# opensensor/thingino-accel

Hardware: AMD Instinct MI355X
Metric: images/sec yolov5s_int8 640x640 batch256 (higher is better)
Workload: dtype int8

## Files before the change

thingino-accel_amd/csrc/hip/conv_i8.hip:

```cpp
#include "conv_i8_common.hpp"

#ifndef I8M_ABL
#define I8M_ABL 0
#endif
template <int BPX, int BN, int STAGES, int KS = 1, int NW = 4>
__global__ __launch_bounds__(NW * 64) void conv_i8_mfma(const mhip_conv_i8_t p, const long total_pix, const int k64,
                                                         const int8_t *__restrict__ zeros, const unsigned noc,
                                                         const unsigned nblk, const int lg_inc, const unsigned kw_magic,
                                                         const fastdiv_t dhw, const fastdiv_t dow, const int bufmode,
                                                         const unsigned in_bytes) {
    ANAT_BEGIN();
    const bool POW2 = lg_inc >= 0;
    const bool masked = p.kh * p.kw <= 32;
    constexpr int SLICE = (BPX + BN) * BK;
    constexpr int STAGE = KS * SLICE;
    constexpr int NWN = BN == 128 ? 2 : 1;
    constexpr int NWM = NW / NWN;
    constexpr int WPX = BPX / NWM / 16;
    constexpr int WOC = BN / NWN / 16;
    constexpr int XROWS = BPX / NW;
    constexpr int XI = XROWS / 16;
    constexpr int LW = (BN / 16 + NW - 1) / NW;
    constexpr int L = XI + LW;
    static_assert(XI >= 1 && XROWS % 16 == 0, "every wave fetches whole 16-row pieces of the pixel tile");
    extern __shared__ __attribute__((aligned(16))) int8_t dynlds[];
    uint8_t *slut = (uint8_t *)dynlds;
    lds_base_must_be_zero(dynlds);
    long *rowoff = (long *)(dynlds + LUTB);
    int8_t *lds = dynlds + BPX * 8 + LUTB;

    const int tid = threadIdx.x, lane = tid & 63;
    const int wv = __builtin_amdgcn_readfirstlane(tid >> 6);
    const unsigned id = xcd_remap(blockIdx.x, nblk);
    const long pix0 = (long)(id / noc) * BPX;
    const int oc0 = (int)(id % noc) * BN;
    const int hw = p.out_h * p.out_w;

    const int wm = wv % NWM, wn = wv / NWM;
    const int pxw = wm * (WPX * 16), ocw = wn * (WOC * 16);
    v4i acc[WOC][WPX];
    init_acc<WPX, WOC>(p, acc, oc0 + ocw);
    if (p.lut2) { if (tid < 128) ((uint32_t *)slut)[tid] = ((const uint32_t *)p.lut2)[tid]; }
    else if (p.lut && tid < 64) ((uint32_t *)slut)[tid] = ((const uint32_t *)p.lut)[tid];
    fill_rowoff<BPX>(p, rowoff, [=](int row) { long q = pix0 + row; return q < total_pix ? q : -1L; }, (unsigned)hw, dhw);

    const int schunk = (lane & 3) ^ (((lane >> 4) & 1) << 1);
    const int8_t *xwin[XI];
    unsigned tapmask[XI];
    int iy0[XI], ix0[XI];
#pragma unroll
    for (int j = 0; j < XI; j++) {
        const long pix = pix0 + wv * XROWS + j * 16 + (lane >> 2);
        const bool valid = pix < total_pix;
        const unsigned f = valid ? fdiv((unsigned)pix, dhw) : 0u;
        const unsigned rem = valid ? (unsigned)pix - f * (unsigned)hw : 0u;
        const int oy = (int)fdiv(rem, dow), ox = (int)(rem - (unsigned)oy * (unsigned)p.out_w);
        iy0[j] = valid ? oy * p.stride_h - p.pad_top : -(1 << 28);
        ix0[j] = ox * p.stride_w - p.pad_left;
        xwin[j] = p.in + (size_t)f * p.in_stride + ((long)iy0[j] * p.in_w + ix0[j]) * p.in_c;
        unsigned m = 0;
        if (masked) {
            const int kx_lo = ix0[j] < 0 ? -ix0[j] : 0, kx_hi = p.in_w - ix0[j] < p.kw ? p.in_w - ix0[j] : p.kw;
            const unsigned colbits = kx_hi > kx_lo ? ((kx_hi >= 32 ? ~0u : (1u << kx_hi) - 1u) & ~((1u << kx_lo) - 1u)) : 0u;
            for (int r = 0; r < p.kh; r++) {
                const int iy = iy0[j] + r;
                if (iy >= 0 && iy < p.in_h) m |= colbits << (r * p.kw);
            }
// ... 57 lines not shown
#pragma unroll
        for (int j = 0; j < XI; j++) {
            bool ok;
            if (masked) {
                ok = kvalid & ((tapmask[j] >> tap) & 1u);
            } else {
                const int iy = iy0[j] + ky, ix = ix0[j] + kx;
                ok = kvalid & (iy >= 0) & (iy < p.in_h) & (ix >= 0) & (ix < p.in_w);
            }
            const int8_t *src = ok ? xwin[j] + koff : zeros;
            glds16(src, sb + (wv * XROWS + j * 16) * BK);
        }
#pragma unroll
        for (int j = 0; j < LW; j++) glds16(wsrc[j] + ks * BK, sb + BPX * BK + wq[j] * 16 * BK);
        if (!POW2) {
            rc += BK;
            while (rc >= p.in_c) { rc -= p.in_c; kx++; }
            while (kx >= p.kw) { kx -= p.kw; ky++; }
        }
    };

    const int nst = I8M_ABL & 2 ? 0 : nks / KS;
#pragma unroll
    for (int s = 0; s < STAGES - 1; s++)
        if (s < nst)
#pragma unroll
            for (int u = 0; u < KS; u++) issue(s * KS + u, s);

    const int frow = lane & 15, fchunk = lane >> 4;
    int stage = 0, nstage = STAGES - 1;
    ANAT_NOW(1);
    for (int st = 0; st < nst; st++) {
        const int ahead = nst - 1 - st;
        if (STAGES >= 4 && ahead >= 2) wait_vmcnt<2 * L * KS>();
        else if (STAGES >= 3 && ahead >= 1) wait_vmcnt<L * KS>();
        else wait_vmcnt<0>();
        __builtin_amdgcn_s_barrier();
        asm volatile("" ::: "memory");
#pragma unroll
        for (int u = 0; u < KS; u++) {
            const int8_t *xs = lds + stage * STAGE + u * SLICE, *ws = xs + BPX * BK;
            v4i xb[WPX], wa[WOC];
#pragma unroll
            for (int t = 0; t < WPX; t++) xb[t] = *(const v4i *)(xs + lds_off(pxw + t * 16 + frow, fchunk));
#pragma unroll
            for (int s = 0; s < WOC; s++) wa[s] = *(const v4i *)(ws + lds_off(ocw + s * 16 + frow, fchunk));
            if (u == 0 && st + STAGES - 1 < nst)
#pragma unroll
                for (int v = 0; v < KS; v++) issue((st + STAGES - 1) * KS + v, nstage);
#pragma unroll
            for (int s = 0; s < WOC; s++)
#pragma unroll
                for (int t = 0; t < WPX; t++) {
                    if (I8M_ABL & 4) asm volatile("" ::"v"(wa[s]), "v"(xb[t]));
                    else acc[s][t] = __builtin_amdgcn_mfma_i32_16x16x64_i8(wa[s], xb[t], acc[s][t], 0, 0, 0);
                }
        }
        stage = stage + 1 == STAGES ? 0 : stage + 1;
        nstage = nstage + 1 == STAGES ? 0 : nstage + 1;
    }
    ANAT_NOW(2);
    __syncthreads();
    if (I8M_ABL & 1) {
        int fold = 0;
#pragma unroll
        for (int s = 0; s < WOC; s++)
#pragma unroll
            for (int t = 0; t < WPX; t++) fold ^= acc[s][t][0] ^ acc[s][t][1] ^ acc[s][t][2] ^ acc[s][t][3];
        if (fold == 0x12345678) p.out[0] = 1;
        return;
    }
    epilogue<BPX, BN, WPX, WOC, true>(p, acc, lds, slut, rowoff, oc0, pxw, ocw, hw);
    ANAT_END(p);
}

__device__ __forceinline__ int lds_off128(int row, int chunk8) { return row * 128 + ((chunk8 ^ ((row >> 1) & 7)) << 4); }
template <int BPX, int BN, int NW>
__global__ __launch_bounds__(NW * 64) void conv_i8_r128(const mhip_conv_i8_t p, const long total_pix, const int k128,
                                                         const unsigned noc, const unsigned nblk, const int lg_inc,
                                                         const unsigned kw_magic, const fastdiv_t dhw, const fastdiv_t dow,
                                                         const unsigned in_bytes) {
    constexpr int STAGE = (BPX + BN) * 128;
    constexpr int NWN = BN == 128 ? 2 : 1;
    constexpr int NWM = NW / NWN;
    constexpr int WPX = BPX / NWM / 16;
    constexpr int WOC = BN / NWN / 16;
    constexpr int XI = BPX / 8 / NW;
    constexpr int WI = BN / 8 / NW;
    static_assert(XI >= 1 && WI >= 1 && BPX % (8 * NW) == 0 && BN % (8 * NW) == 0, "whole 8-row pieces per wave");
    extern __shared__ __attribute__((aligned(16))) int8_t dynlds[];
    uint8_t *slut = (uint8_t *)dynlds;
    lds_base_must_be_zero(dynlds);
    long *rowoff = (long *)(dynlds + LUTB);
    int8_t *lds = dynlds + BPX * 8 + LUTB;

    const int tid = threadIdx.x, lane = tid & 63;
    const int wv = __builtin_amdgcn_readfirstlane(tid >> 6);
    const unsigned id = xcd_remap(blockIdx.x, nblk);
    const long pix0 = (long)(id / noc) * BPX;
    const int oc0 = (int)(id % noc) * BN;
    const int hw = p.out_h * p.out_w;
    const int wm = wv % NWM, wn = wv / NWM;
    const int pxw = wm * (WPX * 16), ocw = wn * (WOC * 16);
    v4i acc[WOC][WPX];
    init_acc<WPX, WOC>(p, acc, oc0 + ocw);
    if (p.lut2) { if (tid < 128) ((uint32_t *)slut)[tid] = ((const uint32_t *)p.lut2)[tid]; }
    else if (p.lut && tid < 64) ((uint32_t *)slut)[tid] = ((const uint32_t *)p.lut)[tid];
    fill_rowoff<BPX>(p, rowoff, [=](int row) { long q = pix0 + row; return q < total_pix ? q : -1L; }, (unsigned)hw, dhw);

    const int lrow = lane >> 3, lslot = lane & 7;
    int xvoff[XI];
    unsigned tapmask[XI];
#pragma unroll
    for (int j = 0; j < XI; j++) {
        const int trow = (wv * XI + j) * 8 + lrow;
        const long pix = pix0 + trow;
        const bool valid = pix < total_pix;
        const unsigned f = valid ? fdiv((unsigned)pix, dhw) : 0u;
        const unsigned rem = valid ? (unsigned)pix - f * (unsigned)hw : 0u;
        const int oy = (int)fdiv(rem, dow), ox = (int)(rem - (unsigned)oy * (unsigned)p.out_w);
        const int iy0 = oy * p.stride_h - p.pad_top, ix0 = ox * p.stride_w - p.pad_left;
        const int chunk = lslot ^ ((trow >> 1) & 7);
        xvoff[j] = (int)(f * (unsigned)p.in_stride) + (iy0 * p.in_w + ix0) * p.in_c + chunk * 16;
        const int kx_lo = ix0 < 0 ? -ix0 : 0, kx_hi = p.in_w - ix0 < p.kw ? p.in_w - ix0 : p.kw;
        const unsigned colbits = kx_hi > kx_lo ? ((kx_hi >= 32 ? ~0u : (1u << kx_hi) - 1u) & ~((1u << kx_lo) - 1u)) : 0u;
        unsigned m = 0;
        for (int r = 0; r < p.kh; r++) {
            const int iy = iy0 + r;
            if (iy >= 0 && iy < p.in_h) m |= colbits << (r * p.kw);
        }
        tapmask[j] = valid ? m : 0u;
// ... 4 lines not shown
        const int trow = (wv * WI + j) * 8 + lrow;
        wvoff[j] = (oc0 + trow) * k128 + (lslot ^ ((trow >> 1) & 7)) * 16;
    }
    const __amdgpu_buffer_rsrc_t xrs = __builtin_amdgcn_make_buffer_rsrc((void *)p.in, 0, (int)in_bytes, 0x00020000);
    const __amdgpu_buffer_rsrc_t wrs = __builtin_amdgcn_make_buffer_rsrc((void *)p.w, 0, p.oc_pad * k128, 0x00020000);
    const int taps = p.kh * p.kw;
    const int nst = k128 / 128;
    auto issue = [&](int st, int buf) {
        int8_t *sb = lds + buf * STAGE;
        const int utap = (st * 128) >> lg_inc, urc = (st * 128) & ((1 << lg_inc) - 1);
        const int uky = (int)(((unsigned)utap * kw_magic) >> 16), ukx = utap - uky * p.kw;
        const int ukoff = (uky * p.in_w + ukx) * p.in_c + urc;
        const bool uvalid = utap < taps;
#pragma unroll
        for (int j = 0; j < XI; j++) {
            const bool ok = uvalid & (((tapmask[j] >> utap) & 1u) != 0u);
            blds16(xrs, ok ? xvoff[j] + ukoff : -1, 0, sb + (wv * XI + j) * 1024);
        }
#pragma unroll
        for (int j = 0; j < WI; j++) blds16(wrs, wvoff[j], st * 128, sb + BPX * 128 + (wv * WI + j) * 1024);
    };

    issue(0, 0);
    const int frow = lane & 15, fchunk = lane >> 4;
    for (int st = 0; st < nst; st++) {
        wait_vmcnt<0>();
        __builtin_amdgcn_s_barrier();
        asm volatile("" ::: "memory");
        const int8_t *xs = lds + (st & 1) * STAGE, *ws = xs + BPX * 128;
        v4i xb[2][WPX], wa[2][WOC];
#pragma unroll
        for (int h = 0; h < 2; h++) {
#pragma unroll
            for (int t = 0; t < WPX; t++) xb[h][t] = *(const v4i *)(xs + lds_off128(pxw + t * 16 + frow, h * 4 + fchunk));
#pragma unroll
            for (int q = 0; q < WOC; q++) wa[h][q] = *(const v4i *)(ws + lds_off128(ocw + q * 16 + frow, h * 4 + fchunk));
        }
        if (st + 1 < nst) issue(st + 1, (st + 1) & 1);
#pragma unroll
        for (int h = 0; h < 2; h++)
#pragma unroll
            for (int q = 0; q < WOC; q++)
#pragma unroll
                for (int t = 0; t < WPX; t++) acc[q][t] = __builtin_amdgcn_mfma_i32_16x16x64_i8(wa[h][q], xb[h][t], acc[q][t], 0, 0, 0);
    }
    __syncthreads();
    epilogue<BPX, BN, WPX, WOC, true>(p, acc, lds, slut, rowoff, oc0, pxw, ocw, hw);
}

template <int A, int B>
__device__ __forceinline__ void wait_vmcnt_at_most(int n) {
    constexpr int HI = A > B ? A : B, LO = A > B ? B : A;
    if (n >= A + B) wait_vmcnt<A + B>();
    else if (n >= HI) wait_vmcnt<HI>();
    else if (n >= LO) wait_vmcnt<LO>();
    else wait_vmcnt<0>();
}

struct conv_out_side_t {
    int8_t *out;
    size_t out_stride;
    const int8_t *w;
    const int32_t *bias;
    const uint8_t *lut, *lut2;
    int out_c, relu, out_pix_stride, out_ch_off;
    float cs;
    unsigned out_bytes;
};
template <int BPX, int BN, int STAGES, bool HAS_LUT, bool SEG = false, bool PAIR = false>
__global__ __launch_bounds__(NTHREADS) void conv_i8_persist(const mhip_conv_i8_t pin, const unsigned total_pix, const int k64,
                                                            const int8_t *__restrict__ zeros, const unsigned noc,
                                                            const unsigned npt, const unsigned ngrp, const int lg_inc,
                                                            const unsigned kw_magic, const fastdiv_t dhw, const fastdiv_t dow,
                                                            const unsigned out_bytes_first, const conv_out_side_t alt,
                                                            const unsigned noc0, const int bufmode, const unsigned in_bytes,
                                                            const int wres) {
    ANAT_BEGIN();
    const int STAGE = wres ? BPX * BK : (BPX + BN) * BK;
    constexpr int NWN = BN == 128 ? 2 : 1;
    constexpr int NWM = 4 / NWN;
    constexpr int WPX = BPX / NWM / 16;
    constexpr int WOC = BN / NWN / 16;
    constexpr int XI = BPX / 64;
    constexpr int LW = BN >= 128 ? 2 : 1;
    constexpr int L = XI + LW;
    constexpr int NST = WPX;
    extern __shared__ __attribute__((aligned(16))) int8_t dynlds[];
    uint8_t *slut = (uint8_t *)dynlds;
    int8_t *lds = dynlds + LUTB;
    lds_base_must_be_zero(dynlds);

    const int tid = threadIdx.x, lane = tid & 63;
    const int wv = __builtin_amdgcn_readfirstlane(tid >> 6);
    const unsigned id = xcd_remap(blockIdx.x, noc * ngrp);
    const unsigned grp = id / noc;
    unsigned ot = id - grp * noc;
    mhip_conv_i8_t p = pin;
    unsigned out_bytes = out_bytes_first;
    if (PAIR && ot >= noc0) {
        ot -= noc0;
        p.lut2 = alt.lut2;
        p.out = alt.out; p.out_stride = alt.out_stride; p.w = alt.w; p.bias = alt.bias; p.lut = alt.lut;
        p.out_c = alt.out_c; p.relu = alt.relu; p.out_pix_stride = alt.out_pix_stride; p.out_ch_off = alt.out_ch_off;
        p.cs = alt.cs;
        out_bytes = alt.out_bytes;
    }
    const int oc0 = (int)ot * BN;
    const unsigned t0 = (unsigned)(((unsigned long long)grp * npt) / ngrp);
    const unsigned t1 = (unsigned)(((unsigned long long)(grp + 1) * npt) / ngrp);
    if (t0 >= t1) return;
    const unsigned hw = (unsigned)(p.out_h * p.out_w);
    const int wm = wv % NWM, wn = wv / NWM;
    const int pxw = wm * (WPX * 16), ocw = wn * (WOC * 16);

    auto packed_row16 = [](int c) { return ((c >> 2) & 1) * 16 + (c >> 3) * 4 + (c & 3); };
    v4i bias[WOC];
#pragma unroll
    for (int s = 0; s < WOC; s++)
        bias[s] = p.bias ? *(const v4i *)(p.bias + (BN == 16 ? packed_row16((lane >> 4) * 4) : oc0 + ocw + s * 16 + (lane >> 4) * 4)) : (v4i){0, 0, 0, 0};
    if (HAS_LUT) {
        if (p.lut2) { if (tid < 128) ((uint32_t *)slut)[tid] = ((const uint32_t *)p.lut2)[tid]; }
        else if (tid < 64) ((uint32_t *)slut)[tid] = ((const uint32_t *)p.lut)[tid];
        __syncthreads();
    }
    const __amdgpu_buffer_rsrc_t orsrc = __builtin_amdgcn_make_buffer_rsrc(p.out, 0, (int)out_bytes, 0x00020000);

    const int schunk = (lane & 3) ^ (((lane >> 4) & 1) << 1);
    const int8_t *xwin[XI];
    unsigned tapmask[XI];
    unsigned rowf[SEG ? XI : 1], rowrem[SEG ? XI : 1];
    unsigned rowrem_up[SEG ? XI : 1];
    int xvoff[XI];
    auto setup_rows = [&](unsigned tile) {
#pragma unroll
        for (int j = 0; j < XI; j++) {
            const unsigned pix = tile * BPX + wv * (BPX / 4) + j * 16 + (lane >> 2);
            const bool valid = pix < total_pix;
            const unsigned f = valid ? fdiv(pix, dhw) : 0u;
            const unsigned rem = valid ? pix - f * hw : 0u;
            if (SEG) {
                rowf[j] = f;
                rowrem[j] = rem;
                const unsigned oy = fdiv(rem, dow), ox = rem - oy * (unsigned)p.out_w;
                rowrem_up[j] = (oy >> 1) * ((unsigned)p.out_w >> 1) + (ox >> 1);
                tapmask[j] = valid ? 1u : 0u;
                continue;
            }
// ... 81 lines not shown
        for (int ks = 0; ks < nks; ks++)
#pragma unroll
            for (int j = 0; j < LW; j++) glds16(wsrc[j] + ks * BK, wres_base + (ks * BN + wq[j] * 16) * BK);
    unsigned itile = t0;
    int iks = 0;
    int younger[STAGES - 1];
    setup_rows(t0);
    int nstage = 0;
#pragma unroll
    for (int s = 0; s < STAGES - 1; s++) {
        int n = 0;
        if (itile < t1) {
            issue(iks, nstage);
            n = wres ? XI : L;
            if (++iks == nks) {
                iks = 0;
                if (++itile < t1) setup_rows(itile);
            }
        }
#pragma unroll
        for (int i = 0; i < s; i++) younger[i] += n;
        younger[s] = 0;
        nstage++;
    }
    nstage = STAGES - 1;

    const int frow = lane & 15, fchunk = lane >> 4;
    const int chan = ocw + (lane >> 4) * (4 * WOC);
    const int pstride = p.out_pix_stride ? p.out_pix_stride : p.out_c;
    const int lo = p.relu ? 0 : -128;
    const uint8_t *lut128 = slut + 128;
    const bool ragged = (p.out_c % (WOC * 4)) != 0;
    int stage = 0;
    ANAT_NOW(1);
    for (unsigned tile = t0; tile < t1; tile++) {
        v4i acc[WOC][WPX];
        for (int ks = 0; ks < nks; ks++) {
            wait_vmcnt_at_most<(STAGES - 2) * L, NST>(younger[0]);
            __builtin_amdgcn_s_barrier();
            asm volatile("" ::: "memory");
            const int8_t *xs = lds + stage * STAGE, *ws = wres ? wres_base + ks * (BN * BK) : xs + BPX * BK;
            v4i xb[WPX], wa[WOC];
#pragma unroll
            for (int t = 0; t < WPX; t++) xb[t] = *(const v4i *)(xs + lds_off(pxw + t * 16 + frow, fchunk));
#pragma unroll
            for (int s = 0; s < WOC; s++) wa[s] = *(const v4i *)(ws + lds_off(ocw + s * 16 + frow, fchunk));
            int n = 0;
            if (itile < t1) {
                issue(iks, nstage);
                n = wres ? XI : L;
                if (++iks == nks) {
                    iks = 0;
                    if (++itile < t1) setup_rows(itile);
                }
            }
#pragma unroll
            for (int i = 0; i + 1 < STAGES - 1; i++) younger[i] = younger[i + 1] + n;
            younger[STAGES - 2] = 0;
            if (ks == 0) {
#pragma unroll
                for (int s = 0; s < WOC; s++)
#pragma unroll
                    for (int t = 0; t < WPX; t++) acc[s][t] = __builtin_amdgcn_mfma_i32_16x16x64_i8(wa[s], xb[t], bias[s], 0, 0, 0);
            } else {
#pragma unroll
                for (int s = 0; s < WOC; s++)
#pragma unroll
                    for (int t = 0; t < WPX; t++) acc[s][t] = __builtin_amdgcn_mfma_i32_16x16x64_i8(wa[s], xb[t], acc[s][t], 0, 0, 0);
            }
            stage = stage + 1 == STAGES ? 0 : stage + 1;
            nstage = nstage + 1 == STAGES ? 0 : nstage + 1;
        }
#ifdef ANATOMY
        if (tile + 1 == t1) ANAT_NOW(2);
#endif
#pragma unroll
        for (int t = 0; t < WPX; t++) {
            const unsigned pix = tile * BPX + pxw + t * 16 + (lane & 15);
            const unsigned f = fdiv(pix, dhw), rem = pix - f * hw;
            const unsigned off = f * (unsigned)p.out_stride + rem * (unsigned)pstride + (unsigned)(p.out_ch_off + oc0 + chan);
            const int nvalid = p.out_c - (oc0 + chan);
            const bool ok = pix < total_pix && nvalid >= WOC * 4;
// ... 217 lines not shown
        if (key && !strcmp(key, e.k)) {
            if (get) *get = *e.v;
            else *e.v = value;
            return 0;
        }
    return -1;
}
extern "C" int mhip_conv_i8_tune(const char *key, int value) { return tune_access(key, value, nullptr); }
extern "C" int mhip_conv_i8_tune_get(const char *key, int *value) { return value ? tune_access(key, 0, value) : -1; }

static int buf_mode(const mhip_conv_i8_t *p, int k64) {
    if (!tune().bufmode) return 0;
    return p->in_c >= 64 && (p->in_c & (p->in_c - 1)) == 0 && p->kh * p->kw <= 32 && (long)p->kh * p->kw * (p->kw - 1) < 65536 &&
           in_extent_bytes(p) <= 0x7fffffffL && (long)p->oc_pad * k64 <= 0x7fffffffL;
}

template <int BPX, int BN, int STAGES, int KS = 1, int NW = 4>
static int launch_mfma(const mhip_conv_i8_t *p, long total_pix, int k64) {
    const unsigned npt = (unsigned)((total_pix + BPX - 1) / BPX), noc = (unsigned)(p->oc_pad / BN);
    const unsigned nblk = npt * noc;
    const int nks = k64 / BK, nst = nks / KS, used = nst < STAGES ? nst : STAGES;
    if (KS > 1 && (nks % KS) != 0) return -1;
    size_t ring = (size_t)used * KS * (BPX + BN) * BK, tile = (size_t)BPX * (BN + OPAD);
    const size_t lds = BPX * 8 + LUTB + (ring > tile ? ring : tile);
    if (lds > 64 * 1024) {
        static bool attr = false;
        if (!attr && hipFuncSetAttribute((const void *)conv_i8_mfma<BPX, BN, STAGES, KS, NW>, hipFuncAttributeMaxDynamicSharedMemorySize,
                                         (int)(BPX * 8 + LUTB + (size_t)STAGES * KS * (BPX + BN) * BK)) != hipSuccess)
            return mhip_check(hipErrorUnknown, "conv_i8_mfma LDS attribute");
        attr = true;
    }
    int lg = -1;
    if ((p->in_c & (p->in_c - 1)) == 0 && (long)p->kh * p->kw * (p->kw - 1) < 65536) {
        lg = 0;
        while ((1 << lg) < p->in_c) lg++;
    }
    const unsigned magic = ((65536u + (unsigned)p->kw - 1u) / (unsigned)p->kw);
    hipLaunchKernelGGL((conv_i8_mfma<BPX, BN, STAGES, KS, NW>), dim3(nblk), dim3(NW * 64), lds, mhip_stream_native(), *p, total_pix,
                       k64, (const int8_t *)mhip_zero_page(), noc, nblk, lg, magic,
                       make_fastdiv((unsigned)(p->out_h * p->out_w)), make_fastdiv((unsigned)p->out_w),
                       lg >= 0 ? buf_mode(p, k64) : 0, (unsigned)in_extent_bytes(p));
    return mhip_check(hipGetLastError(), "conv_i8_mfma launch");
}


template <int BPX, int BN>
static size_t wres_lds(int k64) { return LUTB + 2 * (size_t)BPX * BK + (size_t)(k64 / BK) * BN * BK; }

template <int BPX, int BN, int STAGES, bool HAS_LUT, bool SEG = false, bool PAIR = false>
static int launch_persist_t(const mhip_conv_i8_t *p, long total_pix, int k64, int lg, unsigned magic,
                            const mhip_conv_i8_t *second = nullptr, int wres = 0) {
    if (BN == 16 && (p->out_c > 16 || p->oc_pad != 32 || (PAIR && (second->out_c > 16 || second->oc_pad != 32)))) return -1;
    const unsigned noc0 = BN == 16 ? 1u : (unsigned)(p->oc_pad / BN);
    const unsigned npt = (unsigned)((total_pix + BPX - 1) / BPX), noc = noc0 + (PAIR ? (BN == 16 ? 1u : (unsigned)(second->oc_pad / BN)) : 0u);
    conv_out_side_t alt;
    memset(&alt, 0, sizeof(alt));
    if (PAIR) {
        alt.out = second->out; alt.out_stride = second->out_stride; alt.w = second->w; alt.bias = second->bias;
        alt.lut = second->lut; alt.lut2 = second->lut2; alt.out_c = second->out_c; alt.relu = second->relu; alt.out_pix_stride = second->out_pix_stride;
        alt.out_ch_off = second->out_ch_off; alt.cs = second->cs;
    }
    if (PAIR) alt.out_bytes = (unsigned)persist_out_bytes(second);
    if (wres && STAGES != 2) return -1;
    const size_t lds = wres ? wres_lds<BPX, BN>(k64) : LUTB + (size_t)STAGES * (BPX + BN) * BK;
    if (wres) {
        static bool attr = false;
        if (!attr && hipFuncSetAttribute((const void *)conv_i8_persist<BPX, BN, STAGES, HAS_LUT, SEG, PAIR>,
                                         hipFuncAttributeMaxDynamicSharedMemorySize, 80 * 1024) != hipSuccess)
            return mhip_check(hipErrorUnknown, "conv_i8_persist LDS attribute");
        attr = true;
        int occ = 0, dev = 0;
        hipDeviceProp_t prop;
        if (hipOccupancyMaxActiveBlocksPerMultiprocessor(&occ, conv_i8_persist<BPX, BN, STAGES, HAS_LUT, SEG, PAIR>, NTHREADS, lds) != hipSuccess ||
            hipGetDevice(&dev) != hipSuccess || hipGetDeviceProperties(&prop, dev) != hipSuccess)
            return mhip_check(hipErrorUnknown, "conv_i8_persist occupancy query");
        unsigned g = (unsigned)((occ > 0 ? occ : 1) * prop.multiProcessorCount) / noc;
        if (tune().persist_slots > 0) g = (unsigned)tune().persist_slots / noc;
        if (g < 1) g = 1;
        if (g > npt) g = npt;
        hipLaunchKernelGGL((conv_i8_persist<BPX, BN, STAGES, HAS_LUT, SEG, PAIR>), dim3(noc * g), dim3(NTHREADS), lds,
                           mhip_stream_native(), *p, (unsigned)total_pix, k64, (const int8_t *)mhip_zero_page(), noc, npt, g, lg,
                           magic, make_fastdiv((unsigned)(p->out_h * p->out_w)), make_fastdiv((unsigned)p->out_w),
                           (unsigned)persist_out_bytes(p), alt, noc0, SEG ? 0 : buf_mode(p, k64), (unsigned)in_extent_bytes(p), 1);
        return mhip_check(hipGetLastError(), "conv_i8_persist (resident weights) launch");
    }
    static int slots = 0;
    if (!slots) {
// ... 29 lines not shown
}
static variant_t variant_of(int code) {
    if (code == 20) return variant_t{0, 0, 0, 0, 0, 0, 0, 0, 1};
    if (code == 18 || code == 19) return variant_t{0, 0, 0, 0, 0, 0, 0, code - 17, 0};
    if (code == 14 || code == 15) return variant_t{1, code == 15 ? 256 : 128, 2, 0, 0, 0, 1, 0, 0};
    if (code == 13) return variant_t{0, 256, 3, 0, 0, 1, 0, 0, 0};
    if (code == 12) return variant_t{0, 128, 2, 0, 1, 0, 0, 0, 0};
    if (code >= 9 && code <= 11) return variant_t{0, 0, 0, code == 10 ? 16 : (code == 9 ? 8 : 4), 0, 0, 0, 0, 0};
    if (code > 8 || code == 6 || code == 8) return variant_t{-1, 0, 0, 0, 0, 0, 0, 0, 0};
    const int c = code - 1;
    return variant_t{c & 1, (c & 2) ? 256 : 128, (c & 4) ? 3 : 2, 0, 0, 0, 0, 0, 0};
}

static bool r128_ok(const mhip_conv_i8_t *p) {
    const int C = p->in_c;
    return C >= 128 && (C & (C - 1)) == 0 && p->oc_pad % 128 == 0 && p->kh * p->kw <= 32 && (long)p->kh * p->kw * (p->kw - 1) < 65536 &&
           p->row_pad == p->kw * C && p->nseg <= 1 && in_extent_bytes(p) <= 0x7fffffffL && (long)p->oc_pad * p->kh * p->row_pad <= 0x7fffffffL;
}
template <int BPX, int BN, int NW>
static int launch_r128_t(const mhip_conv_i8_t *p, long total_pix) {
    const int k128 = p->kh * p->row_pad;
    const unsigned npt = (unsigned)((total_pix + BPX - 1) / BPX), noc = (unsigned)(p->oc_pad / BN);
    size_t ring = 2 * (size_t)(BPX + BN) * 128, tile = (size_t)BPX * (BN + OPAD);
    const size_t lds = BPX * 8 + LUTB + (ring > tile ? ring : tile);
    static bool attr = false;
    if (!attr && hipFuncSetAttribute((const void *)conv_i8_r128<BPX, BN, NW>, hipFuncAttributeMaxDynamicSharedMemorySize, (int)lds) != hipSuccess)
        return mhip_check(hipErrorUnknown, "conv_i8_r128 LDS attribute");
    attr = true;
    int lg = 0;
    while ((1 << lg) < p->in_c) lg++;
    const unsigned magic = ((65536u + (unsigned)p->kw - 1u) / (unsigned)p->kw);
    hipLaunchKernelGGL((conv_i8_r128<BPX, BN, NW>), dim3(npt * noc), dim3(NW * 64), lds, mhip_stream_native(), *p, total_pix, k128, noc,
                       npt * noc, lg, magic, make_fastdiv((unsigned)(p->out_h * p->out_w)), make_fastdiv((unsigned)p->out_w),
                       (unsigned)in_extent_bytes(p));
    return mhip_check(hipGetLastError(), "conv_i8_r128 launch");
}
static int launch_r128(const mhip_conv_i8_t *p, long total_pix, int form) {
    if (!r128_ok(p)) return -1;
    return form == 2 ? launch_r128_t<256, 128, 8>(p, total_pix) : launch_r128_t<128, 128, 4>(p, total_pix);
}
static bool seg_valid(const mhip_conv_i8_t *p) {
    if (p->nseg < 2 || p->nseg > 4 || p->kh != 1 || p->kw != 1 || p->stride_h != 1 || p->stride_w != 1 || p->pad_top ||
        p->pad_left || p->in_h != p->out_h || p->in_w != p->out_w)
        return false;
    int c = 0;
    if (p->seg_up && ((p->out_h | p->out_w) & 1)) return false;
    if (p->seg_up >> p->nseg) return false;
    for (int i = 0; i < 4; i++) {
        if (i < p->nseg) {
            if (!p->seg_in[i] || p->seg_c[i] <= 0 || (p->seg_c[i] & 31) || p->seg_c0[i] != c) return false;
            c += p->seg_c[i];
        } else if (p->seg_c0[i] != 0x7fffffff) {
            return false;
        }
    }
    return c == p->in_c;
}
static bool persist_eligible(const mhip_conv_i8_t *p) {
    if (p->add) return false;
    return !p->out_nchw && p->safe && (p->in_c & (p->in_c - 1)) == 0 && p->kh * p->kw <= 32 &&
           (long)p->kh * p->kw * (p->kw - 1) < 65536 && persist_out_bytes(p) <= 0x7fffffffL;
}
static bool wres_default(const mhip_conv_i8_t *p, int nks, int *bpx) {
    if (!tune().wres || p->kh * p->kw != 1 || p->in_c < 64 || p->out_h * p->out_w > 6400) return false;
    const int bn = p->oc_pad % 128 == 0 ? 128 : (p->oc_pad % 64 == 0 ? 64 : 32);
    const int px = (bn == 64 && p->out_h * p->out_w >= 6400) ? 256 : 128;
    if (LUTB + 2 * (size_t)px * BK + (size_t)nks * bn * BK > 80 * 1024) return false;
    *bpx = px;
    return true;
}

static variant_t default_variant(const mhip_conv_i8_t *p, int nks) {
    variant_t v;
    v.patch = 0;
    v.ks2 = 0;
    v.w8 = 0;
    v.wres = 0;
    v.r128 = 0;
    v.rows = 0;
    int ring = 0;
    const long wg_large = ((long)p->frames * p->out_h * p->out_w + 255) / 256 * ((p->oc_pad + 127) / 128);
    const bool few = wg_large < tune().few_wgs && tune().persist && !tune().bpx && !tune().stages && tune().small_batch;
    if (few) {
        if (conv_i8_patch_ok(p, 4, &ring)) {
            v.persist = 0; v.bpx = 0; v.stages = 0; v.patch = 4;
            return v;
        }
        if (nks >= 8 && r128_ok(p)) {
            v.persist = 0; v.bpx = 0; v.stages = 0; v.r128 = 1;
            return v;
// ... 133 lines not shown

extern "C" int mhip_conv_i8_variants(const mhip_conv_i8_t *p, int *codes, int max) {
    if (!p || (p->in_c % 16) != 0 || mhip_conv_i8_small_c(p->in_c, p->kw, p->out_c)) return 0;
    const int k64 = (p->kh * p->row_pad + BK - 1) / BK * BK, nks = k64 / BK;
    int n = 0;
    if (p->pre_w) {
        const int first = conv_i8_pre_tile_rows(p);
        for (int th : {first, 16, 8, 4})
            if (th && n < max && conv_i8_patch_ok(p, th, nullptr)) {
                const int code = th == 16 ? 10 : (th == 8 ? 9 : 11);
                bool seen = false;
                for (int i = 0; i < n; i++) seen |= codes[i] == code;
                if (!seen) codes[n++] = code;
            }
        return n;
    }
    if (p->nseg > 1) {
        const int bn = p->oc_pad % 128 == 0 ? 128 : (p->oc_pad % 64 == 0 ? 64 : 32);
        const variant_t dv = default_variant(p, nks);
        const int dflt = dv.persist && dv.wres ? (dv.bpx == 256 ? 15 : 14) : (dv.bpx == 256 ? 4 : 2);
        if (n < max) codes[n++] = dflt;
        if (n < max && dflt != 2) codes[n++] = 2;
        if (n < max && dflt != 4) codes[n++] = 4;
        if (n < max && dflt != 14 && LUTB + 2 * (size_t)128 * BK + (size_t)nks * bn * BK <= 80 * 1024) codes[n++] = 14;
        if (n < max && dflt != 15 && LUTB + 2 * (size_t)256 * BK + (size_t)nks * bn * BK <= 80 * 1024) codes[n++] = 15;
        return n;
    }
    const int dflt = variant_code(default_variant(p, nks));
    if (n < max) codes[n++] = dflt;
    for (int code = 1; code <= NVARIANTS; code++) {
        const variant_t v = variant_of(code);
        if (code == dflt) continue;
        if (v.patch && !conv_i8_patch_ok(p, v.patch, nullptr)) continue;
        if (v.persist && !persist_eligible(p)) continue;
        if (v.ks2 && ((nks & 1) || nks < 4 || p->oc_pad % 64 != 0)) continue;
        if (v.w8 && (p->oc_pad % 128 != 0 || nks < 3)) continue;
        if (v.persist < 0) continue;
        if (v.r128 && !r128_ok(p)) continue;
        if (v.rows && !conv_i8_rows_ok(p)) continue;
        if (v.wres) {
            const int bn = p->oc_pad % 128 == 0 ? 128 : (p->oc_pad % 64 == 0 ? 64 : 32);
            if (LUTB + 2 * (size_t)v.bpx * BK + (size_t)nks * bn * BK > 80 * 1024) continue;
        }
        if (!v.persist && v.stages == 3 && nks <= 2) continue;
        if (n < max) codes[n++] = code;
    }
    return n;
}

template <int BN>
static int launch_generic(const mhip_conv_i8_t *p, long total_pix, int k64) {
    dim3 grid((unsigned)((total_pix + BP - 1) / BP), (unsigned)(p->oc_pad / BN));
    hipLaunchKernelGGL((conv_i8_generic<BN>), grid, dim3(NTHREADS), 0, mhip_stream_native(), *p, total_pix, k64,
                       make_fastdiv((unsigned)(p->out_h * p->out_w)));
    return mhip_check(hipGetLastError(), "conv_i8_generic launch");
}

extern "C" int mhip_conv_i8(const mhip_conv_i8_t *p) {
    if (!p || !p->in || !p->out || !p->w) return -1;
    if (p->out_pix_stride < 0 || p->out_ch_off < 0 || (p->out_nchw && (p->out_pix_stride || p->out_ch_off)) ||
        (p->out_pix_stride && p->out_pix_stride < p->out_ch_off + p->out_c))
        return -1;
    if (p->frames <= 0 || p->in_h <= 0 || p->in_w <= 0 || p->in_c <= 0 || p->out_h <= 0 || p->out_w <= 0 ||
        p->out_c <= 0 || p->kh <= 0 || p->kw <= 0 || p->stride_h < 0 || p->stride_w < 0)
        return -1;
// ... 72 lines not shown
```

thingino-accel_amd/csrc/hip/conv_i8_common.hpp:

```cpp
#pragma once
#include <hip/hip_runtime.h>
#include <stdint.h>
#include <stdlib.h>
#include <string.h>
#include <type_traits>

#include "../mhip.h"

extern "C" hipStream_t mhip_stream_native(void);
extern "C" int mhip_check(hipError_t e, const char *what);
extern "C" const void *mhip_zero_page(void);

typedef int v4i __attribute__((ext_vector_type(4)));
typedef int v2i __attribute__((ext_vector_type(2)));

#ifdef ANATOMY
struct anat_rec_t {
    unsigned key, wg, hwid, xcc;
    unsigned long long t[4];
};
static __device__ anat_rec_t *g_anat_buf;
static __device__ unsigned g_anat_cap;
#define ANAT_SETTER(NAME)                                                                                                    \
    extern "C" int NAME(void *buf, unsigned cap) {                                                                          \
        return hipMemcpyToSymbol(HIP_SYMBOL(g_anat_buf), &buf, sizeof buf) == hipSuccess &&                                  \
                       hipMemcpyToSymbol(HIP_SYMBOL(g_anat_cap), &cap, sizeof cap) == hipSuccess                             \
                   ? 0                                                                                                       \
                   : -1;                                                                                                     \
    }
#define ANAT_NOW(i)                                                                                                          \
    do {                                                                                                                     \
        __builtin_amdgcn_sched_barrier(0);                                                                                   \
        an_t[i] = __builtin_amdgcn_s_memrealtime();                                                                          \
        __builtin_amdgcn_sched_barrier(0);                                                                                   \
    } while (0)
#define ANAT_BEGIN()                                                                                                         \
    unsigned long long an_t[4] = {0, 0, 0, 0};                                                                               \
    ANAT_NOW(0)
#define ANAT_END(P)                                                                                                          \
    do {                                                                                                                     \
        ANAT_NOW(3);                                                                                                         \
        if (threadIdx.x == 0 && g_anat_buf) {                                                                                \
            const unsigned an_i = atomicAdd(&g_anat_buf[0].key, 1u) + 1u;                                                    \
            if (an_i < g_anat_cap) {                                                                                         \
                anat_rec_t an_r;                                                                                             \
                an_r.key = (unsigned)((size_t)(P).out >> 4) ^ (unsigned)(P).out_ch_off;                                      \
                an_r.wg = blockIdx.x + gridDim.x * blockIdx.y;                                                               \
                an_r.hwid = __builtin_amdgcn_s_getreg(4 | (0 << 6) | (31 << 11));        \
                an_r.xcc = __builtin_amdgcn_s_getreg(20 | (0 << 6) | (3 << 11));                                 \
                for (int q = 0; q < 4; q++) an_r.t[q] = an_t[q];                                                             \
                g_anat_buf[an_i] = an_r;                                                                                     \
            }                                                                                                                \
        }                                                                                                                    \
    } while (0)
#else
#define ANAT_SETTER(NAME)
#define ANAT_NOW(i) do { } while (0)
#define ANAT_BEGIN() do { } while (0)
#define ANAT_END(P) do { } while (0)
#endif

#define BP 128
#define BK 64
#define NTHREADS 256
#define OPAD 4
#define LUTB 512

__device__ __forceinline__ int lds_off(int row, int chunk) {
    return row * BK + (((chunk ^ ((row >> 1) & 2))) << 4);
}

template <bool SAFE>
__device__ __forceinline__ int requant(int acc, float cs, int lo) {
    const float scaled = (float)acc * cs;
    const float half = __int_as_float((__float_as_int(scaled) & (int)0x80000000) | 0x3f000000);
    const float biased = scaled + half;
    int r = (int)biased;
    if (!SAFE) r = biased < 2147483648.0f ? r : INT_MIN;
    r = r < lo ? lo : r;
    r = r > 127 ? 127 : r;
    return r;
}

__device__ __forceinline__ int requant_safe(int acc, float cs, int lo, int hi) {
    const float scaled = (float)acc * cs;
    const float half = __int_as_float((__float_as_int(scaled) & (int)0x80000000) | 0x3f000000);
    const int r = (int)(scaled + half);
    int m;
    asm("v_med3_i32 %0, %1, %2, %3" : "=v"(m) : "v"(r), "v"(lo), "v"(hi));
// ... 276 lines not shown
    const bool direct = !p.out_nchw && ((p.out_c | p.out_pix_stride | p.out_ch_off) & 15) == 0;
#define EPI(L, S, D) epilogue_t<BPX, BN, WPX, WOC, L, S, D, LUT0>(p, acc, tile, slut, rowoff, oc0, pxw, ocw, hw)
    if (direct) {
        if (p.lut) { if (p.safe) EPI(true, true, true); else EPI(true, false, true); }
        else { if (p.safe) EPI(false, true, true); else EPI(false, false, true); }
    } else {
        if (p.lut) { if (p.safe) EPI(true, true, false); else EPI(true, false, false); }
        else { if (p.safe) EPI(false, true, false); else EPI(false, false, false); }
    }
#undef EPI
}

template <int WPX, int WOC>
__device__ __forceinline__ void init_acc(const mhip_conv_i8_t &p, v4i (&acc)[WOC][WPX], int ocbase) {
    const int lane = threadIdx.x & 63;
#pragma unroll
    for (int s = 0; s < WOC; s++) {
        const v4i b = p.bias ? *(const v4i *)(p.bias + ocbase + s * 16 + (lane >> 4) * 4) : (v4i){0, 0, 0, 0};
#pragma unroll
        for (int t = 0; t < WPX; t++) acc[s][t] = b;
    }
}


struct tune_t {
    int init;
    int persist;
    int persist_stages;
    int persist_maxk;
    int persist_slots;
    int stages;
    int bpx;
    int variant;
    int bufmode;
    int small_batch;
    int rgb_direct;
    int wres;
    int few_wgs;
    int rows;
    int patch_ring;
    int patch_lds_kb;
};
const tune_t &conv_i8_tune_state();

extern "C" int mhip_conv_i8_small_c(int in_c, int kw, int out_c);

// ... 19 lines not shown
```

Baseline: 57830.

## Stage LUT and bias tables via async global-to-LDS DMA overlapped with prologue

Result: no change. 57540 (-0.5%).

```diff
diff --git a/thingino-accel_amd/csrc/hip/conv_i8.hip b/thingino-accel_amd/csrc/hip/conv_i8.hip
--- a/thingino-accel_amd/csrc/hip/conv_i8.hip
+++ b/thingino-accel_amd/csrc/hip/conv_i8.hip
@@ -26,8 +26,8 @@
     extern __shared__ __attribute__((aligned(16))) int8_t dynlds[];
     uint8_t *slut = (uint8_t *)dynlds;
     lds_base_must_be_zero(dynlds);
-    long *rowoff = (long *)(dynlds + LUTB);
-    int8_t *lds = dynlds + BPX * 8 + LUTB;
+    long *rowoff = (long *)(dynlds + TABB);
+    int8_t *lds = dynlds + BPX * 8 + TABB;
 
     const int tid = threadIdx.x, lane = tid & 63;
     const int wv = __builtin_amdgcn_readfirstlane(tid >> 6);
@@ -39,10 +39,7 @@
     const int wm = wv % NWM, wn = wv / NWM;
     const int pxw = wm * (WPX * 16), ocw = wn * (WOC * 16);
     v4i acc[WOC][WPX];
-    init_acc<WPX, WOC>(p, acc, oc0 + ocw);
-    if (p.lut2) { if (tid < 128) ((uint32_t *)slut)[tid] = ((const uint32_t *)p.lut2)[tid]; }
-    else if (p.lut && tid < 64) ((uint32_t *)slut)[tid] = ((const uint32_t *)p.lut)[tid];
-    fill_rowoff<BPX>(p, rowoff, [=](int row) { long q = pix0 + row; return q < total_pix ? q : -1L; }, (unsigned)hw, dhw);
+    ANAT_NOW(4);
 
     const int schunk = (lane & 3) ^ (((lane >> 4) & 1) << 1);
     const int8_t *xwin[XI];
@@ -146,10 +143,23 @@
 
     const int nst = I8M_ABL & 2 ? 0 : nks / KS;
 #pragma unroll
-    for (int s = 0; s < STAGES - 1; s++)
+    for (int s = 0; s < STAGES - 1; s++) {
         if (s < nst)
 #pragma unroll
             for (int u = 0; u < KS; u++) issue(s * KS + u, s);
+        if (s == 0) {
+            ANAT_NOW(6);
+            stage_tables(p.lut, p.lut2, p.bias, oc0, BN, zeros, dynlds);
+            ANAT_NOW(5);
+        }
+    }
+    fill_rowoff<BPX>(p, rowoff, [=](int row) { long q = pix0 + row; return q < total_pix ? q : -1L; }, (unsigned)hw, dhw);
+    if (I8M_ABL & 2) {
+#pragma unroll
+        for (int s = 0; s < WOC; s++)
+#pragma unroll
+            for (int t = 0; t < WPX; t++) acc[s][t] = (v4i){0, 0, 0, 0};
+    }
 
     const int frow = lane & 15, fchunk = lane >> 4;
     int stage = 0, nstage = STAGES - 1;
@@ -159,6 +169,9 @@
         if (STAGES >= 4 && ahead >= 2) wait_vmcnt<2 * L * KS>();
         else if (STAGES >= 3 && ahead >= 1) wait_vmcnt<L * KS>();
         else wait_vmcnt<0>();
+#ifdef ANATOMY
+        if (st == 0) ANAT_NOW(7);
+#endif
         __builtin_amdgcn_s_barrier();
         asm volatile("" ::: "memory");
 #pragma unroll
@@ -172,13 +185,25 @@
             if (u == 0 && st + STAGES - 1 < nst)
 #pragma unroll
                 for (int v = 0; v < KS; v++) issue((st + STAGES - 1) * KS + v, nstage);
-#pragma unroll
-            for (int s = 0; s < WOC; s++)
-#pragma unroll
-                for (int t = 0; t < WPX; t++) {
-                    if (I8M_ABL & 4) asm volatile("" ::"v"(wa[s]), "v"(xb[t]));
-                    else acc[s][t] = __builtin_amdgcn_mfma_i32_16x16x64_i8(wa[s], xb[t], acc[s][t], 0, 0, 0);
-                }
+            if (st == 0 && u == 0) {
+                v4i bias[WOC];
+                bias_from_lds<WOC>(dynlds, bias, ocw);
+#pragma unroll
+                for (int s = 0; s < WOC; s++)
+#pragma unroll
+                    for (int t = 0; t < WPX; t++) {
+                        if (I8M_ABL & 4) { asm volatile("" ::"v"(wa[s]), "v"(xb[t])); acc[s][t] = bias[s]; }
+                        else acc[s][t] = __builtin_amdgcn_mfma_i32_16x16x64_i8(wa[s], xb[t], bias[s], 0, 0, 0);
+                    }
+            } else {
+#pragma unroll
+                for (int s = 0; s < WOC; s++)
+#pragma unroll
+                    for (int t = 0; t < WPX; t++) {
+                        if (I8M_ABL & 4) asm volatile("" ::"v"(wa[s]), "v"(xb[t]));
+                        else acc[s][t] = __builtin_amdgcn_mfma_i32_16x16x64_i8(wa[s], xb[t], acc[s][t], 0, 0, 0);
+                    }
+            }
         }
         stage = stage + 1 == STAGES ? 0 : stage + 1;
         nstage = nstage + 1 == STAGES ? 0 : nstage + 1;
@@ -203,7 +228,7 @@
 __global__ __launch_bounds__(NW * 64) void conv_i8_r128(const mhip_conv_i8_t p, const long total_pix, const int k128,
                                                          const unsigned noc, const unsigned nblk, const int lg_inc,
                                                          const unsigned kw_magic, const fastdiv_t dhw, const fastdiv_t dow,
-                                                         const unsigned in_bytes) {
+                                                         const unsigned in_bytes, const int8_t *__restrict__ zeros) {
     constexpr int STAGE = (BPX + BN) * 128;
     constexpr int NWN = BN == 128 ? 2 : 1;
     constexpr int NWM = NW / NWN;
@@ -215,8 +240,8 @@
     extern __shared__ __attribute__((aligned(16))) int8_t dynlds[];
     uint8_t *slut = (uint8_t *)dynlds;
     lds_base_must_be_zero(dynlds);
-    long *rowoff = (long *)(dynlds + LUTB);
-    int8_t *lds = dynlds + BPX * 8 + LUTB;
+    long *rowoff = (long *)(dynlds + TABB);
+    int8_t *lds = dynlds + BPX * 8 + TABB;
 
     const int tid = threadIdx.x, lane = tid & 63;
     const int wv = __builtin_amdgcn_readfirstlane(tid >> 6);
@@ -227,10 +252,6 @@
     const int wm = wv % NWM, wn = wv / NWM;
     const int pxw = wm * (WPX * 16), ocw = wn * (WOC * 16);
     v4i acc[WOC][WPX];
-    init_acc<WPX, WOC>(p, acc, oc0 + ocw);
-    if (p.lut2) { if (tid < 128) ((uint32_t *)slut)[tid] = ((const uint32_t *)p.lut2)[tid]; }
-    else if (p.lut && tid < 64) ((uint32_t *)slut)[tid] = ((const uint32_t *)p.lut)[tid];
-    fill_rowoff<BPX>(p, rowoff, [=](int row) { long q = pix0 + row; return q < total_pix ? q : -1L; }, (unsigned)hw, dhw);
 
     const int lrow = lane >> 3, lslot = lane & 7;
     int xvoff[XI];
@@ -281,6 +302,8 @@
     };
 
     issue(0, 0);
+    stage_tables(p.lut, p.lut2, p.bias, oc0, BN, zeros, dynlds);
+    fill_rowoff<BPX>(p, rowoff, [=](int row) { long q = pix0 + row; return q < total_pix ? q : -1L; }, (unsigned)hw, dhw);
     const int frow = lane & 15, fchunk = lane >> 4;
     for (int st = 0; st < nst; st++) {
         wait_vmcnt<0>();
@@ -296,12 +319,23 @@
             for (int q = 0; q < WOC; q++) wa[h][q] = *(const v4i *)(ws + lds_off128(ocw + q * 16 + frow, h * 4 + fchunk));
         }
         if (st + 1 < nst) issue(st + 1, (st + 1) & 1);
-#pragma unroll
-        for (int h = 0; h < 2; h++)
+        if (st == 0) {
+            v4i bias[WOC];
+            bias_from_lds<WOC>(dynlds, bias, ocw);
 #pragma unroll
             for (int q = 0; q < WOC; q++)
 #pragma unroll
-                for (int t = 0; t < WPX; t++) acc[q][t] = __builtin_amdgcn_mfma_i32_16x16x64_i8(wa[h][q], xb[h][t], acc[q][t], 0, 0, 0);
+                for (int t = 0; t < WPX; t++) acc[q][t] = __builtin_amdgcn_mfma_i32_16x16x64_i8(wa[0][q], xb[0][t], bias[q], 0, 0, 0);
+        } else {
+#pragma unroll
+            for (int q = 0; q < WOC; q++)
+#pragma unroll
+                for (int t = 0; t < WPX; t++) acc[q][t] = __builtin_amdgcn_mfma_i32_16x16x64_i8(wa[0][q], xb[0][t], acc[q][t], 0, 0, 0);
+        }
+#pragma unroll
+        for (int q = 0; q < WOC; q++)
+#pragma unroll
+            for (int t = 0; t < WPX; t++) acc[q][t] = __builtin_amdgcn_mfma_i32_16x16x64_i8(wa[1][q], xb[1][t], acc[q][t], 0, 0, 0);
     }
     __syncthreads();
     epilogue<BPX, BN, WPX, WOC, true>(p, acc, lds, slut, rowoff, oc0, pxw, ocw, hw);
@@ -346,7 +380,7 @@
     constexpr int NST = WPX;
     extern __shared__ __attribute__((aligned(16))) int8_t dynlds[];
     uint8_t *slut = (uint8_t *)dynlds;
-    int8_t *lds = dynlds + LUTB;
+    int8_t *lds = dynlds + TABB;
     lds_base_must_be_zero(dynlds);
 
     const int tid = threadIdx.x, lane = tid & 63;
@@ -373,15 +407,8 @@
     const int pxw = wm * (WPX * 16), ocw = wn * (WOC * 16);
 
     auto packed_row16 = [](int c) { return ((c >> 2) & 1) * 16 + (c >> 3) * 4 + (c & 3); };
-    v4i bias[WOC];
-#pragma unroll
-    for (int s = 0; s < WOC; s++)
-        bias[s] = p.bias ? *(const v4i *)(p.bias + (BN == 16 ? packed_row16((lane >> 4) * 4) : oc0 + ocw + s * 16 + (lane >> 4) * 4)) : (v4i){0, 0, 0, 0};
-    if (HAS_LUT) {
-        if (p.lut2) { if (tid < 128) ((uint32_t *)slut)[tid] = ((const uint32_t *)p.lut2)[tid]; }
-        else if (tid < 64) ((uint32_t *)slut)[tid] = ((const uint32_t *)p.lut)[tid];
-        __syncthreads();
-    }
+    static_assert(STAGES == 2, "the first wait of the K stream must cover the tables: they are the newest DMA of the prologue");
+    ANAT_NOW(4);
     const __amdgpu_buffer_rsrc_t orsrc = __builtin_amdgcn_make_buffer_rsrc(p.out, 0, (int)out_bytes, 0x00020000);
 
     const int schunk = (lane & 3) ^ (((lane >> 4) & 1) << 1);
@@ -509,6 +536,12 @@
         for (int i = 0; i < s; i++) younger[i] += n;
         younger[s] = 0;
         nstage++;
+        if (s == 0) {
+            ANAT_NOW(6);
+            stage_tables(HAS_LUT ? p.lut : nullptr, HAS_LUT ? p.lut2 : nullptr, p.bias, oc0, BN == 16 ? 32 : BN, zeros, dynlds);
+            younger[0] += 1;
+            ANAT_NOW(5);
+        }
     }
     nstage = STAGES - 1;
 
@@ -524,6 +557,9 @@
         v4i acc[WOC][WPX];
         for (int ks = 0; ks < nks; ks++) {
             wait_vmcnt_at_most<(STAGES - 2) * L, NST>(younger[0]);
+#ifdef ANATOMY
+            if (tile == t0 && ks == 0) ANAT_NOW(7);
+#endif
             __builtin_amdgcn_s_barrier();
             asm volatile("" ::: "memory");
             const int8_t *xs = lds + stage * STAGE, *ws = wres ? wres_base + ks * (BN * BK) : xs + BPX * BK;
@@ -545,6 +581,10 @@
             for (int i = 0; i + 1 < STAGES - 1; i++) younger[i] = younger[i + 1] + n;
             younger[STAGES - 2] = 0;
             if (ks == 0) {
+                v4i bias[WOC];
+#pragma unroll
+                for (int s = 0; s < WOC; s++)
+                    bias[s] = *(const v4i *)(dynlds + LUTB + (BN == 16 ? packed_row16((lane >> 4) * 4) : ocw + s * 16 + (lane >> 4) * 4) * 4);
 #pragma unroll
                 for (int s = 0; s < WOC; s++)
 #pragma unroll
@@ -808,11 +848,11 @@
     const int nks = k64 / BK, nst = nks / KS, used = nst < STAGES ? nst : STAGES;
     if (KS > 1 && (nks % KS) != 0) return -1;
     size_t ring = (size_t)used * KS * (BPX + BN) * BK, tile = (size_t)BPX * (BN + OPAD);
-    const size_t lds = BPX * 8 + LUTB + (ring > tile ? ring : tile);
+    const size_t lds = BPX * 8 + TABB + (ring > tile ? ring : tile);
     if (lds > 64 * 1024) {
         static bool attr = false;
         if (!attr && hipFuncSetAttribute((const void *)conv_i8_mfma<BPX, BN, STAGES, KS, NW>, hipFuncAttributeMaxDynamicSharedMemorySize,
-                                         (int)(BPX * 8 + LUTB + (size_t)STAGES * KS * (BPX + BN) * BK)) != hipSuccess)
+                                         (int)(BPX * 8 + TABB + (size_t)STAGES * KS * (BPX + BN) * BK)) != hipSuccess)
             return mhip_check(hipErrorUnknown, "conv_i8_mfma LDS attribute");
         attr = true;
     }
@@ -831,7 +871,7 @@
 
 
 template <int BPX, int BN>
-static size_t wres_lds(int k64) { return LUTB + 2 * (size_t)BPX * BK + (size_t)(k64 / BK) * BN * BK; }
+static size_t wres_lds(int k64) { return TABB + 2 * (size_t)BPX * BK + (size_t)(k64 / BK) * BN * BK; }
 
 template <int BPX, int BN, int STAGES, bool HAS_LUT, bool SEG = false, bool PAIR = false>
 static int launch_persist_t(const mhip_conv_i8_t *p, long total_pix, int k64, int lg, unsigned magic,
@@ -848,7 +888,7 @@
     }
     if (PAIR) alt.out_bytes = (unsigned)persist_out_bytes(second);
     if (wres && STAGES != 2) return -1;
-    const size_t lds = wres ? wres_lds<BPX, BN>(k64) : LUTB + (size_t)STAGES * (BPX + BN) * BK;
+    const size_t lds = wres ? wres_lds<BPX, BN>(k64) : TABB + (size_t)STAGES * (BPX + BN) * BK;
     if (wres) {
         static bool attr = false;
         if (!attr && hipFuncSetAttribute((const void *)conv_i8_persist<BPX, BN, STAGES, HAS_LUT, SEG, PAIR>,
@@ -924,7 +964,7 @@
     const int k128 = p->kh * p->row_pad;
     const unsigned npt = (unsigned)((total_pix + BPX - 1) / BPX), noc = (unsigned)(p->oc_pad / BN);
     size_t ring = 2 * (size_t)(BPX + BN) * 128, tile = (size_t)BPX * (BN + OPAD);
-    const size_t lds = BPX * 8 + LUTB + (ring > tile ? ring : tile);
+    const size_t lds = BPX * 8 + TABB + (ring > tile ? ring : tile);
     static bool attr = false;
     if (!attr && hipFuncSetAttribute((const void *)conv_i8_r128<BPX, BN, NW>, hipFuncAttributeMaxDynamicSharedMemorySize, (int)lds) != hipSuccess)
         return mhip_check(hipErrorUnknown, "conv_i8_r128 LDS attribute");
@@ -934,7 +974,7 @@
     const unsigned magic = ((65536u + (unsigned)p->kw - 1u) / (unsigned)p->kw);
     hipLaunchKernelGGL((conv_i8_r128<BPX, BN, NW>), dim3(npt * noc), dim3(NW * 64), lds, mhip_stream_native(), *p, total_pix, k128, noc,
                        npt * noc, lg, magic, make_fastdiv((unsigned)(p->out_h * p->out_w)), make_fastdiv((unsigned)p->out_w),
-                       (unsigned)in_extent_bytes(p));
+                       (unsigned)in_extent_bytes(p), (const int8_t *)mhip_zero_page());
     return mhip_check(hipGetLastError(), "conv_i8_r128 launch");
 }
 static int launch_r128(const mhip_conv_i8_t *p, long total_pix, int form) {
@@ -967,7 +1007,7 @@
     if (!tune().wres || p->kh * p->kw != 1 || p->in_c < 64 || p->out_h * p->out_w > 6400) return false;
     const int bn = p->oc_pad % 128 == 0 ? 128 : (p->oc_pad % 64 == 0 ? 64 : 32);
     const int px = (bn == 64 && p->out_h * p->out_w >= 6400) ? 256 : 128;
-    if (LUTB + 2 * (size_t)px * BK + (size_t)nks * bn * BK > 80 * 1024) return false;
+    if (TABB + 2 * (size_t)px * BK + (size_t)nks * bn * BK > 80 * 1024) return false;
     *bpx = px;
     return true;
 }
@@ -1147,8 +1187,8 @@
         if (n < max) codes[n++] = dflt;
         if (n < max && dflt != 2) codes[n++] = 2;
         if (n < max && dflt != 4) codes[n++] = 4;
-        if (n < max && dflt != 14 && LUTB + 2 * (size_t)128 * BK + (size_t)nks * bn * BK <= 80 * 1024) codes[n++] = 14;
-        if (n < max && dflt != 15 && LUTB + 2 * (size_t)256 * BK + (size_t)nks * bn * BK <= 80 * 1024) codes[n++] = 15;
+        if (n < max && dflt != 14 && TABB + 2 * (size_t)128 * BK + (size_t)nks * bn * BK <= 80 * 1024) codes[n++] = 14;
+        if (n < max && dflt != 15 && TABB + 2 * (size_t)256 * BK + (size_t)nks * bn * BK <= 80 * 1024) codes[n++] = 15;
         return n;
     }
     const int dflt = variant_code(default_variant(p, nks));
@@ -1165,7 +1205,7 @@
         if (v.rows && !conv_i8_rows_ok(p)) continue;
         if (v.wres) {
             const int bn = p->oc_pad % 128 == 0 ? 128 : (p->oc_pad % 64 == 0 ? 64 : 32);
-            if (LUTB + 2 * (size_t)v.bpx * BK + (size_t)nks * bn * BK > 80 * 1024) continue;
+            if (TABB + 2 * (size_t)v.bpx * BK + (size_t)nks * bn * BK > 80 * 1024) continue;
         }
         if (!v.persist && v.stages == 3 && nks <= 2) continue;
         if (n < max) codes[n++] = code;
diff --git a/thingino-accel_amd/csrc/hip/conv_i8_common.hpp b/thingino-accel_amd/csrc/hip/conv_i8_common.hpp
--- a/thingino-accel_amd/csrc/hip/conv_i8_common.hpp
+++ b/thingino-accel_amd/csrc/hip/conv_i8_common.hpp
@@ -17,7 +17,7 @@
 #ifdef ANATOMY
 struct anat_rec_t {
     unsigned key, wg, hwid, xcc;
-    unsigned long long t[4];
+    unsigned long long t[8];
 };
 static __device__ anat_rec_t *g_anat_buf;
 static __device__ unsigned g_anat_cap;
@@ -35,7 +35,7 @@
         __builtin_amdgcn_sched_barrier(0);                                                                                   \
     } while (0)
 #define ANAT_BEGIN()                                                                                                         \
-    unsigned long long an_t[4] = {0, 0, 0, 0};                                                                               \
+    unsigned long long an_t[8] = {0, 0, 0, 0, 0, 0, 0, 0};                                                                               \
     ANAT_NOW(0)
 #define ANAT_END(P)                                                                                                          \
     do {                                                                                                                     \
@@ -48,7 +48,7 @@
                 an_r.wg = blockIdx.x + gridDim.x * blockIdx.y;                                                               \
                 an_r.hwid = __builtin_amdgcn_s_getreg(4 | (0 << 6) | (31 << 11));        \
                 an_r.xcc = __builtin_amdgcn_s_getreg(20 | (0 << 6) | (3 << 11));                                 \
-                for (int q = 0; q < 4; q++) an_r.t[q] = an_t[q];                                                             \
+                for (int q = 0; q < 8; q++) an_r.t[q] = an_t[q];                                                             \
                 g_anat_buf[an_i] = an_r;                                                                                     \
             }                                                                                                                \
         }                                                                                                                    \
@@ -65,6 +65,8 @@
 #define NTHREADS 256
 #define OPAD 4
 #define LUTB 512
+#define BIASB 512
+#define TABB (LUTB + BIASB)
 
 __device__ __forceinline__ int lds_off(int row, int chunk) {
     return row * BK + (((chunk ^ ((row >> 1) & 2))) << 4);
@@ -387,6 +389,25 @@
     }
 }
 
+__device__ __forceinline__ void stage_tables(const uint8_t *lut, const uint8_t *lut2, const int32_t *bias, int oc0, int bn,
+                                             const int8_t *zeros, void *lds0) {
+    const int lane = threadIdx.x & 63, l = lane & 31;
+    const uint8_t *tab = lut2 ? lut2 : lut;
+    const int tabn = lut2 ? 32 : (lut ? 16 : 0);
+    const void *src = zeros;
+    if (lane < 32) { if (l < tabn) src = tab + l * 16; }
+    else if (bias && l * 4 < bn) src = bias + oc0 + l * 4;
+    glds16(src, lds0);
+}
+template <int WOC>
+__device__ __forceinline__ void bias_from_lds(const int8_t *lds0, v4i (&b)[WOC], int ocw) {
+    int z = 0;
+    asm volatile("" : "+v"(z));
+    const int lane = (int)__builtin_amdgcn_mbcnt_hi(~0u, __builtin_amdgcn_mbcnt_lo(~0u, (unsigned)z));
+#pragma unroll
+    for (int s = 0; s < WOC; s++) b[s] = *(const v4i *)(lds0 + LUTB + (ocw + s * 16 + (lane >> 4) * 4) * 4);
+}
+
 
 struct tune_t {
     int init;
```
